# HugoNip/ORB_SLAM2_test

Hardware: AMD Instinct MI355X
Metric: frames/sec ORB extract+match, 1241×376 2000feat 8lvl, 1/2/4/8 GPU (higher is better)
Workload: dtype u8; 1 GPU; C3 KITTI03-shaped mono 1241x376, 2000 feat, 8 lvl: ORBextractor + Hamming knn2 (t vs t-1) + SearchForInitialization(w=100, 0.9, checkOri); global_batch=1024, width=1241, pipelined_batches=True, serial_pass_only=False, input_blocks=4, height=376, nfeatures=2000, nlevels=8

## Files before the change

orb_slam2_test_amd/csrc/blur_device.h:

```cpp
#pragma once

#include <hip/hip_runtime.h>

#include "orbg_internal.h"
#include "orbg_device.h"

#pragma clang fp contract(off)

namespace orbg {

#define BLUR2_TW 244
#define BLUR2_TW_T 240
#ifndef BLUR2_LDS_ROW
#define BLUR2_LDS_ROW 68
#endif
#ifndef ORBG_BLUR2_SEG
#define ORBG_BLUR2_SEG 32
#endif
#ifndef ORBG_BLUR2_ROWPF
#define ORBG_BLUR2_ROWPF 4
#endif

__device__ __forceinline__ uint32_t b2_udot2(uint32_t a, uint32_t b, uint32_t c)
{
    typedef unsigned short u16x2 __attribute__((ext_vector_type(2)));
    return __builtin_amdgcn_udot2(__builtin_bit_cast(u16x2, a), __builtin_bit_cast(u16x2, b), c,
                                  false);
}

__device__ __forceinline__ int b2_reflect101(int i, int n)
{
    i = i < 0 ? -i : i;
    return i >= n ? 2 * n - 2 - i : i;
}

struct Blur2Weights {
    uint32_t K00, K01, K10, K11, K12, K20, K21, K22, K31, K32, E0, E1, E2, k6, c0;
    bool norm256;
    __device__ Blur2Weights(const OrbgGeom *g)
    {
        const uint32_t k0 = g->gk[0], k1 = g->gk[1], k2 = g->gk[2], k3 = g->gk[3],
                       k4 = g->gk[4], k5 = g->gk[5];
        k6 = g->gk[6];
        norm256 = k0 + k1 + k2 + k3 + k4 + k5 + k6 == 256u;
        K00 = k0 << 8 | k1 << 16 | k2 << 24;
        K01 = k3 | k4 << 8 | k5 << 16 | k6 << 24;
        K10 = k0 << 16 | k1 << 24;
        K11 = k2 | k3 << 8 | k4 << 16 | k5 << 24;
        K12 = k6;
        K20 = k0 << 24;
        K21 = k1 | k2 << 8 | k3 << 16 | k4 << 24;
        K22 = k5 | k6 << 8;
        K31 = k0 | k1 << 8 | k2 << 16 | k3 << 24;
        K32 = k4 | k5 << 8 | k6 << 16;
        E0 = k0 | k1 << 16;
        E1 = k2 | k3 << 16;
        E2 = k4 | k5 << 16;
        c0 = norm256 ? (1u << 15) : 0u;
    }
};

template <int SEG, bool NORM256, typename Loader, typename Store>
__device__ __forceinline__ void blur2_column(const Blur2Weights &k, Loader &&load, Store &&store)
{
    constexpr int NR = SEG + 6;
    uint32_t s[NR][4];
    uint32_t P[NR][4];
#pragma unroll
    for (int i = 0; i < NR; i++) {
        uint32_t w0, w1, w2;
        load(i, w0, w1, w2);
        s[i][0] = __builtin_amdgcn_udot4(w1, k.K01, __builtin_amdgcn_udot4(w0, k.K00, 0u, false), false);
        s[i][1] = __builtin_amdgcn_udot4(w2, k.K12, __builtin_amdgcn_udot4(w1, k.K11, __builtin_amdgcn_udot4(w0, k.K10, 0u, false), false), false);
        s[i][2] = __builtin_amdgcn_udot4(w2, k.K22, __builtin_amdgcn_udot4(w1, k.K21, __builtin_amdgcn_udot4(w0, k.K20, 0u, false), false), false);
        s[i][3] = __builtin_amdgcn_udot4(w2, k.K32, __builtin_amdgcn_udot4(w1, k.K31, 0u, false), false);
        if (i >= 1) {
#pragma unroll
            for (int c = 0; c < 4; c++) P[i - 1][c] = s[i - 1][c] | s[i][c] << 16;
        }
        if (i >= 6) {
            const int o = i - 6;
            uint32_t a[4];
#pragma unroll
            for (int c = 0; c < 4; c++) {
                uint32_t v = b2_udot2(P[o][c], k.E0, k.c0);
                v = b2_udot2(P[o + 2][c], k.E1, v);
                v = b2_udot2(P[o + 4][c], k.E2, v);
                a[c] = __umul24(k.k6, s[o + 6][c]) + v;
            }
            uint32_t word;
            if constexpr (NORM256) {
                word = __builtin_amdgcn_perm(a[1], a[0], 0x0c0c0602u) |
                       __builtin_amdgcn_perm(a[3], a[2], 0x06020c0cu);
            } else {
                word = 0;
#pragma unroll
                for (int c = 0; c < 4; c++) word |= min((a[c] + (1u << 15)) >> 16, 255u) << (8 * c);
            }
            store(o, word);
        }
    }
}

template <int SEG, bool TILED = false>
__device__ __forceinline__ void blur2_tile(const Blur2Weights &k, const uint8_t *src, int pitch,
                                           int W, int H, uint8_t *dst, int dpitch, int tx, int y0,
                                           int yend, int lane, uint32_t *wlds = nullptr)
{
    constexpr int PF = ORBG_BLUR2_ROWPF;
    constexpr int TW = TILED ? BLUR2_TW_T : BLUR2_TW;
    static_assert(!TILED || SEG % 8 == 0, "tiled output: whole tile rows per wave");
    const int gx = tx * TW + 4 * lane;
    const bool owner = 4 * lane < TW && gx < W;
    const bool left_wave = tx == 0, right_wave = (tx + 1) * TW + 8 > W;
    const bool is_left = gx == 0;
    const int m = W - gx;
    uint32_t sel1 = 0x07060504u, sel2 = 0x07060504u;
    bool pair_lo = false;
    if (m >= 1 && m <= 7) {
        pair_lo = m <= 3;
        sel1 = sel2 = 0;
#pragma unroll
        for (int b = 4; b < 12; b++) {
            int sb = b < m + 4 ? b : 2 * m + 6 - b;
            if (b >= 8) sb = pair_lo ? max(sb, 0) : max(sb, 4) - 4;
            else sb = max(sb, 0);
            if (b < 8) sel1 |= (uint32_t)sb << (8 * (b - 4));
            else sel2 |= (uint32_t)sb << (8 * (b - 8));
        }
    }
    const int nrec = (H - 1) * pitch + W;
    const int sh0 = (int)((uintptr_t)src & 3);
    const __amdgpu_buffer_rsrc_t rsrc = __builtin_amdgcn_make_buffer_rsrc(
        (void *)(src - sh0), (short)0, nrec + sh0, 0x00020000);
    bool strad_wave;
    {
        const int ro = (H - 1) * pitch;
        const int ol = ro - ((ro + sh0) & 3) + gx - 4;
        strad_wave = __ballot(ol + 4 > nrec && ol < nrec) != 0;
    }
    const __amdgpu_buffer_rsrc_t drsrc = __builtin_amdgcn_make_buffer_rsrc(
        (void *)dst, (short)0, (TILED ? (yend + 7) & ~7 : yend) * dpitch, 0x00020000);
    const int lane_off = owner ? gx : (1 << 30);
    const bool interior = y0 >= 3 && y0 + SEG + 3 < H;
    auto run = [&](auto INTERIOR, auto NORM) {
        constexpr bool inner = decltype(INTERIOR)::value;
        uint32_t ring[PF], rsh[PF];
        auto issue = [&](int i) {
            const int y = inner ? y0 - 3 + i : b2_reflect101(min(y0 - 3 + i, H + 2), H);
            const int rowoff = y * pitch;
            const int sh = __builtin_amdgcn_readfirstlane((rowoff + sh0) & 3);
            const int o = rowoff - sh + gx - 4;
            uint32_t v;
            v = __builtin_amdgcn_raw_buffer_load_b32(rsrc, o + sh0, 0, 0);
            if (!inner && strad_wave && y == H - 1) {
                if (o + 4 > nrec && o < nrec) {
                    uint32_t vb = 0;
                    for (int b = 0; b < 4 && o + b < nrec; b++)
                        vb |= (uint32_t)__builtin_amdgcn_raw_buffer_load_b8(rsrc, o + b + sh0, 0, 0) << (8 * b);
                    v = vb;
                }
            }
            ring[i % PF] = v;
            rsh[i % PF] = (uint32_t)sh;
        };
#pragma unroll
        for (int i = 0; i < PF; i++) issue(i);
        blur2_column<SEG, decltype(NORM)::value>(
            k,
            [&](int i, uint32_t &w0, uint32_t &w1, uint32_t &w2) {
                const uint32_t d0 = ring[i % PF], sh = rsh[i % PF];
                if (i + PF < SEG + 6) issue(i + PF);
                const uint32_t d1 = __builtin_amdgcn_mov_dpp(d0, 0x130, 0xF, 0xF, true);
                const uint32_t d2 = __builtin_amdgcn_mov_dpp(d1, 0x130, 0xF, 0xF, true);
                const uint32_t d3 = __builtin_amdgcn_mov_dpp(d2, 0x130, 0xF, 0xF, true);
                w0 = __builtin_amdgcn_alignbyte(d1, d0, sh);
                w1 = __builtin_amdgcn_alignbyte(d2, d1, sh);
                w2 = __builtin_amdgcn_alignbyte(d3, d2, sh);
                if (left_wave) {
                    const uint32_t r = __builtin_amdgcn_perm(w2, w1, 0x01020304u);
                    w0 = is_left ? r : w0;
                }
                if (right_wave) {
                    const uint32_t v1 = __builtin_amdgcn_perm(w1, w0, sel1);
                    const uint32_t v2 = pair_lo ? __builtin_amdgcn_perm(w1, w0, sel2)
                                                : __builtin_amdgcn_perm(w2, w1, sel2);
                    w1 = v1;
                    w2 = v2;
                }
            },
            [&](int o, uint32_t word) {
                if (!TILED) {
                    __builtin_amdgcn_raw_buffer_store_b32(word, drsrc, lane_off + (y0 + o) * dpitch,
                                                          0, 0);
                    return;
                }
                wlds[(o & 7) * BLUR2_LDS_ROW + lane] = word;
                if ((o & 7) != 7) return;
                wave_sync_lds();
                const int tyoff = ((y0 + (o & ~7)) >> 3) * (8 * dpitch);
#pragma unroll
                for (int h = 0; h < 2; h++) {
                    const int idx = lane + 64 * h, t = idx >> 3, r = idx & 7;
                    typedef uint32_t b2_v4u __attribute__((ext_vector_type(4)));
                    const b2_v4u v = *(const b2_v4u *)(wlds + r * BLUR2_LDS_ROW + 4 * t);
                    const int x = tx * TW + 16 * t;
                    const int off = (t < TW / 16 && x < W) ? tyoff + (x >> 4) * 128 + r * 16 : (1 << 30);
                    __builtin_amdgcn_raw_buffer_store_b128(v, drsrc, off, 0, 0);
                }
                wave_sync_lds();
            });
    };
    if (k.norm256) {
        if (interior)
            run(std::true_type{}, std::true_type{});
        else
            run(std::false_type{}, std::true_type{});
    } else {
        if (interior)
            run(std::true_type{}, std::false_type{});
        else
            run(std::false_type{}, std::false_type{});
    }
}

}
```

orb_slam2_test_amd/csrc/match_kernels.hip:

```cpp
#include <hip/hip_runtime.h>

#include <algorithm>
#include <climits>

#include "../../include/orbg.h"
#include "orbg_internal.h"
#include "orbg_device.h"
#include "match_device.h"

#pragma clang fp contract(off)

namespace orbg {

void prof_begin(void *prof, hipStream_t s, const char *n, hipEvent_t *a);
void prof_end(void *prof, hipStream_t s, const char *n, hipEvent_t a);
bool prof_skip_name(const char *n);

#ifndef ORBG_ROW16_SHFL
__device__ __forceinline__ int row16_sum(int x)
{
    x += __builtin_amdgcn_mov_dpp(x, 0x128, 0xf, 0xf, false);
    x += __builtin_amdgcn_mov_dpp(x, 0x124, 0xf, 0xf, false);
    x += __builtin_amdgcn_mov_dpp(x, 0x4e, 0xf, 0xf, false);
    x += __builtin_amdgcn_mov_dpp(x, 0xb1, 0xf, 0xf, false);
    return x;
}
__device__ __forceinline__ unsigned long long row16_min_u64(unsigned long long v)
{
    auto step = [&](auto CTRL) {
        constexpr int c = decltype(CTRL)::value;
        const uint32_t lo = __builtin_amdgcn_mov_dpp((int)(uint32_t)v, c, 0xf, 0xf, false);
        const uint32_t hi = __builtin_amdgcn_mov_dpp((int)(uint32_t)(v >> 32), c, 0xf, 0xf, false);
        const unsigned long long u = (unsigned long long)hi << 32 | lo;
        v = u < v ? u : v;
    };
    step(std::integral_constant<int, 0x128>{});
    step(std::integral_constant<int, 0x124>{});
    step(std::integral_constant<int, 0x4e>{});
    step(std::integral_constant<int, 0xb1>{});
    return v;
}
#else
__device__ __forceinline__ int row16_sum(int x)
{
#pragma unroll
    for (int o = 8; o > 0; o >>= 1) x += __shfl_xor(x, o, 16);
    return x;
}
__device__ __forceinline__ unsigned long long row16_min_u64(unsigned long long mn)
{
#pragma unroll
    for (int o = 8; o > 0; o >>= 1) {
        const unsigned long long u = __shfl_xor(mn, o, 16);
        mn = u < mn ? u : mn;
    }
    return mn;
}
#endif

#define TH_LOW 50
#define HISTO_LENGTH 30

typedef int knn_v4i __attribute__((ext_vector_type(4)));
typedef int knn_v16i __attribute__((ext_vector_type(16)));

#define KNN_MAX_TRAIN 8192
#define KNN_NONE 0x40000000

__device__ __forceinline__ void knn_key_update(int key, int &k1, int &k2)
{
    k2 = min(k2, max(k1, key));
    k1 = min(k1, key);
}

typedef int knn_v8i __attribute__((ext_vector_type(8)));
typedef float knn_v16f __attribute__((ext_vector_type(16)));
#ifndef ORBG_KNN_MED3
#define ORBG_KNN_MED3 1
#endif
#define KNN4_ROWB 144
#define KNN4_SCALE_A (127 + 12)
#define KNN4_SCALE_B 127

__device__ __forceinline__ uint32_t knn4_neg(uint32_t x, int q)
{
    return (((x >> q) & 0x11111111u) << 3) | 0x22222222u;
}
__device__ __forceinline__ uint32_t knn4_pos(uint32_t x, int q)
{
    return knn4_neg(x, q) ^ 0x88888888u;
}

__device__ __forceinline__ void knn2_block_fp4(const uint8_t *__restrict__ q, int nq,
                                               const uint8_t *__restrict__ t, int nt,
                                               int32_t *__restrict__ out, int qbase)
{
    __shared__ __attribute__((aligned(16))) uint8_t tile[2][64 * KNN4_ROWB];
    const int tid = threadIdx.x, lane = tid & 63, wv = tid >> 6;
    const int col = lane & 31, h = lane >> 5;
    knn_v8i bq[2][4];
#pragma unroll
    for (int u = 0; u < 2; u++) {
        const int qi = qbase + wv * 64 + u * 32 + col;
        uint32_t x[4] = {0, 0, 0, 0};
        if (qi < nq) {
            const uint32_t *p = (const uint32_t *)(q + (size_t)qi * 32);
#pragma unroll
            for (int s = 0; s < 4; s++) x[s] = p[2 * s + h];
        }
#pragma unroll
        for (int s = 0; s < 4; s++) {
#pragma unroll
            for (int qd = 0; qd < 4; qd++) {
                bq[u][s][qd] = (int)knn4_pos(x[s], qd);
                bq[u][s][qd + 4] = 0;
            }
        }
    }
    uint32_t k1[2] = {UINT_MAX, UINT_MAX}, k2[2] = {UINT_MAX, UINT_MAX};

    const int er = tid >> 3, esd = tid & 7;
    auto fetch1 = [&](int row) -> uint32_t {
        return ((const uint32_t *)(t + (size_t)min(row, nt - 1) * 32))[esd];
    };
    auto expand1 = [&](uint32_t x, uint8_t *dst) {
        uint4 w;
        w.x = knn4_neg(x, 0); w.y = knn4_neg(x, 1);
        w.z = knn4_neg(x, 2); w.w = knn4_neg(x, 3);
        *(uint4 *)dst = w;
    };
    auto expand = [&](uint32_t x0, uint32_t x1, int bf) {
        expand1(x0, tile[bf] + er * KNN4_ROWB + esd * 16);
        expand1(x1, tile[bf] + (er + 32) * KNN4_ROWB + esd * 16);
    };
    uint32_t xr0 = 0, xr1 = 0;
    if (nt > 0) {
        expand(fetch1(er), fetch1(er + 32), 0);
        xr0 = fetch1(64 + er);
        xr1 = fetch1(96 + er);
    }
    knn_v16f accA[2], accB[2];
    auto epilogue = [&](const knn_v16f (&acc)[2]) {
#pragma unroll
        for (int r = 0; r < 16; r++) {
#pragma unroll
            for (int u = 0; u < 2; u++) {
                const float kf = acc[u][r];
                const uint32_t key = __float_as_uint(kf);
#if ORBG_KNN_MED3
                const uint32_t k1o = k1[u];
                k1[u] = min(k1o, key);
                asm volatile("v_med3_u32 %0, %1, %2, %3" : "=v"(k2[u]) : "v"(k1o), "v"(k2[u]), "v"(key));
#else
                k2[u] = min(k2[u], max(k1[u], key));
                k1[u] = min(k1[u], key);
#endif
            }
        }
    };
    auto subtile = [&](int tb, int bf, int sub, knn_v16f (&acc)[2]) {
        knn_v16f ctag;
        const float tbh = (float)(tb + 4 * h + (1 << 20));
#pragma unroll
        for (int r = 0; r < 16; r++) ctag[r] = tbh + (float)((r & 3) + 8 * (r >> 2));
        if (tb + 32 > nt) {
#pragma unroll
            for (int r = 0; r < 16; r++)
                if (ctag[r] >= (float)(nt + (1 << 20))) ctag[r] = (float)KNN_NONE;
        }
        const uint8_t *arow = tile[bf] + (32 * sub + col) * KNN4_ROWB + h * 16;
#pragma unroll
        for (int s = 0; s < 4; s++) {
            const knn_v4i a4 = *(const knn_v4i *)(arow + s * 32);
            const knn_v8i a = {a4[0], a4[1], a4[2], a4[3], 0, 0, 0, 0};
            acc[0] = __builtin_amdgcn_mfma_scale_f32_32x32x64_f8f6f4(
                a, bq[0][s], s ? acc[0] : ctag, 4, 4, 0, KNN4_SCALE_A, 0, KNN4_SCALE_B);
            acc[1] = __builtin_amdgcn_mfma_scale_f32_32x32x64_f8f6f4(
                a, bq[1][s], s ? acc[1] : ctag, 4, 4, 0, KNN4_SCALE_A, 0, KNN4_SCALE_B);
        }
    };
    bool pendB = false;
    for (int s0 = 0, bf = 0; s0 < nt; s0 += 64, bf ^= 1) {
        __syncthreads();
        if (s0 + 64 < nt) {
            expand(xr0, xr1, bf ^ 1);
            xr0 = fetch1(s0 + 128 + er);
            xr1 = fetch1(s0 + 160 + er);
        }
        subtile(s0, bf, 0, accA);
        if (pendB) epilogue(accB);
        pendB = s0 + 32 < nt;
        if (pendB) subtile(s0 + 32, bf, 1, accB);
        epilogue(accA);
    }
    if (pendB) epilogue(accB);
    const uint32_t none = 0x4E000000u;
#pragma unroll
    for (int u = 0; u < 2; u++) {
        const uint32_t o1 = (uint32_t)__shfl_xor((int)k1[u], 32, 64);
        const uint32_t o2 = (uint32_t)__shfl_xor((int)k2[u], 32, 64);
        const uint32_t b1 = min(k1[u], o1);
        const uint32_t b2 = min(min(k2[u], o2), max(k1[u], o1));
        const int qi = qbase + wv * 64 + u * 32 + col;
        if (h == 0 && qi < nq) {
            const bool v1 = b1 < none, v2 = b2 < none;
            const int e1 = v1 ? (int)__builtin_bit_cast(float, b1) : 0;
            const int e2 = v2 ? (int)__builtin_bit_cast(float, b2) : 0;
            out[(size_t)qi * 3 + 0] = v1 ? (e1 & (KNN_MAX_TRAIN - 1)) : -1;
            out[(size_t)qi * 3 + 1] = v1 ? (e1 >> 13) : INT_MAX;
            out[(size_t)qi * 3 + 2] = v2 ? (e2 >> 13) : INT_MAX;
        }
    }
}

__global__ __launch_bounds__(256) __attribute__((amdgpu_waves_per_eu(4, 8))) void k_knn2_single(
    const uint8_t *q, int nq, const uint8_t *t, int nt, int32_t *out)
{
    knn2_block_fp4(q, nq, t, nt, out, blockIdx.x * 256);
}

#define KNN2_PAIRS_BODY(BLOCK)                                                                 \
    const int nbx = (fc + 255) >> 8;                                                           \
    const int id = xcd_remap(blockIdx.x, gridDim.x);                                           \
    const int p = id / nbx, bx = id - p * nbx;                                                 \
    const int a = f1[p], b = f2[p];                                                            \
    const int nq = counts[b], nt = counts[a];                                                  \
    if (bx * 256 >= nq) return;                                                                \
    BLOCK(desc + (size_t)b * fc * 32, nq, desc + (size_t)a * fc * 32, nt,                      \
          out + (size_t)p * fc * 3, bx * 256);
__global__ __launch_bounds__(256) __attribute__((amdgpu_waves_per_eu(4, 8))) void k_knn2_pairs(
    const uint8_t *desc, const int32_t *counts, int fc, const int32_t *f1, const int32_t *f2,
    int32_t *out)
{
    KNN2_PAIRS_BODY(knn2_block_fp4)
}

struct F2Key {
    float x, y;
    int idx;
};

#ifndef INIT_QPW
#define INIT_QPW 8
#endif
#ifndef INIT_QPW_SINGLE
#define INIT_QPW_SINGLE 4
#endif
#define INIT_F2_CAP 4608

__host__ __device__ constexpr size_t init_cands_keys_bytes(int f2cap)
{
    return ((size_t)2 * f2cap * sizeof(F2Key) + 15) & ~(size_t)15;
}
#ifndef ORBG_INIT_LDSD
#define ORBG_INIT_LDSD 1
#endif
__host__ __device__ constexpr bool init_cands_lds(int f2cap)
{
    return ORBG_INIT_LDSD && init_cands_keys_bytes(f2cap) + (size_t)f2cap * 32 <= 65536;
}

template <bool LDSD, int QPW>
__device__ __forceinline__ void init_cands_block(const orbg_keypoint *__restrict__ k1,
                                 const uint8_t *__restrict__ d1, int n1,
                                 const orbg_keypoint *__restrict__ k2,
                                 const uint8_t *__restrict__ d2, int n2, orbg_bounds b,
                                 const float *__restrict__ prev, int prev_stride, int window,
                                 unsigned long long *__restrict__ topk, int32_t *__restrict__ topn,
                                 int qbase, int f2cap)
{
    extern __shared__ __attribute__((aligned(16))) F2Key f2mem[];
    F2Key *f2raw = f2mem, *f2 = f2mem + f2cap;
    uint4 *d2l = (uint4 *)((uint8_t *)f2mem + init_cands_keys_bytes(f2cap));
    __shared__ int nf2;
    __shared__ int colstart[ORBG_GRID_COLS + 1];
    const int tid = threadIdx.x, lane = tid & 63, wv = tid >> 6;
    const GridPrm g = grid_prm(b);
    if (tid == 0) nf2 = 0;
    if (tid <= ORBG_GRID_COLS) colstart[tid] = 0;
    __syncthreads();
    const int n2s = min(n2, f2cap);
    if (LDSD) {
        const uint4 *src = (const uint4 *)d2;
        for (int i0 = 0; i0 < 2 * n2s; i0 += 4 * 256) {
            uint4 v[4];
#pragma unroll
            for (int u = 0; u < 4; u++) {
                const int i = i0 + u * 256 + tid;
                v[u] = src[i < 2 * n2s ? i : 0];
            }
#pragma unroll
            for (int u = 0; u < 4; u++) {
                const int i = i0 + u * 256 + tid;
                if (i < 2 * n2s) d2l[i] = v[u];
            }
        }
    }
    for (int i = tid; i < n2s; i += 256) {
        const orbg_keypoint kp = k2[i];
        if (kp.octave == 0) {
            const int px = (int)roundf((kp.x - g.min_x) * g.inv_w);
            if (px < 0 || px >= ORBG_GRID_COLS) continue;
            const int s = atomicAdd(&nf2, 1);
            if (s < f2cap) {
                f2raw[s] = F2Key{kp.x, kp.y, i};
                atomicAdd(&colstart[px + 1], 1);
            }
        }
    }
    __syncthreads();
    const int m = min(nf2, f2cap);
    if (wv == 0) {
        const int c = colstart[lane + 1];
        const int incl = wave_incl_scan(c);
        colstart[lane + 1] = incl;
    }
    __syncthreads();
    __shared__ int cursor[ORBG_GRID_COLS];
    if (tid < ORBG_GRID_COLS) cursor[tid] = colstart[tid];
    __syncthreads();
    for (int j = tid; j < m; j += 256) {
        const F2Key fk = f2raw[j];
        const int px = (int)roundf((fk.x - g.min_x) * g.inv_w);
        f2[atomicAdd(&cursor[px], 1)] = fk;
    }
    __syncthreads();
    const float r = (float)window;
    const int grp = lane >> 4, sub = lane & 15;
    for (int qq = 0; qq < QPW; qq += 4) {
        const int i1 = qbase + wv * QPW + qq + grp;
        bool act = i1 < n1;
        if (act && k1[i1].octave > 0) {
            if (sub == 0) topn[i1] = -1;
            act = false;
        }
        if (!__any(act)) continue;
        unsigned long long loc[ORBG_MATCH_TOPK];
#pragma unroll
        for (int k = 0; k < ORBG_MATCH_TOPK; k++) loc[k] = ~0ull;
        int cnt = 0;
        if (act) {
            const Window w = make_window(g, prev[(size_t)i1 * prev_stride],
                                         prev[(size_t)i1 * prev_stride + 1], r);
            uint32_t qd[8];
            {
                const uint4 *p = (const uint4 *)(d1 + (size_t)i1 * 32);
                const uint4 a = p[0], c = p[1];
                qd[0] = a.x; qd[1] = a.y; qd[2] = a.z; qd[3] = a.w;
                qd[4] = c.x; qd[5] = c.y; qd[6] = c.z; qd[7] = c.w;
            }
            if (!w.empty) {
                const int j0 = colstart[w.cx0], j1 = colstart[w.cx1 + 1];
                for (int j = j0 + sub; j < j1; j += 16) {
                    const F2Key fk = f2[j];
                    const int ord = cand_order(g, w, fk.x, fk.y);
                    if (ord < 0) continue;
                    const int d = LDSD ? hamming8(qd, (const uint32_t *)(d2l + 2 * fk.idx))
                                       : hamming8(qd, (const uint32_t *)(d2 + (size_t)fk.idx * 32));
                    unsigned long long key = ((unsigned long long)d << 32) |
                                             ((unsigned long long)ord << 20) | (unsigned)fk.idx;
                    cnt++;
#pragma unroll
                    for (int k = 0; k < ORBG_MATCH_TOPK; k++) {
                        const unsigned long long lo = key < loc[k] ? key : loc[k];
                        const unsigned long long hi = key < loc[k] ? loc[k] : key;
                        loc[k] = lo;
                        key = hi;
                    }
                }
            }
        }
        cnt = row16_sum(cnt);
        int head = 0;
        unsigned long long *out = topk + (size_t)i1 * ORBG_MATCH_TOPK;
        for (int k = 0; k < ORBG_MATCH_TOPK; k++) {
            unsigned long long mine = ~0ull;
#pragma unroll
            for (int h = 0; h < ORBG_MATCH_TOPK; h++)
                if (h == head) mine = loc[h];
            const unsigned long long mn = row16_min_u64(mine);
            if (mn != ~0ull && mine == mn) head++;
            if (act && sub == 0) out[k] = mn;
        }
        if (act && sub == 0) topn[i1] = cnt;
    }
}

template <bool LDSD>
__global__ __launch_bounds__(256) void k_init_cands_single(
    const orbg_keypoint *k1, const uint8_t *d1, int n1, const orbg_keypoint *k2,
    const uint8_t *d2, int n2, orbg_bounds b, const float *prev, int window,
    unsigned long long *topk, int32_t *topn)
{
    init_cands_block<LDSD, INIT_QPW_SINGLE>(k1, d1, n1, k2, d2, n2, b, prev, 2, window, topk, topn,
                                            blockIdx.x * 4 * INIT_QPW_SINGLE, n2);
}

template <bool LDSD>
__global__ __launch_bounds__(256) void k_init_cands_pairs(
    const orbg_keypoint *kps, const uint8_t *desc, const int32_t *counts, int fc,
    const int32_t *f1, const int32_t *f2, orbg_bounds b, int window, unsigned long long *topk,
    int32_t *topn, int cap)
{
    const int nbx = (cap + 4 * INIT_QPW - 1) / (4 * INIT_QPW);
    const int id = xcd_remap(blockIdx.x, gridDim.x);
    const int p = id / nbx, bx = id - p * nbx;
    const int a = f1[p], c = f2[p];
    const int n1 = counts[a], n2 = counts[c];
    const int qbase = bx * 4 * INIT_QPW;
    if (qbase >= n1) return;
    const orbg_keypoint *k1 = kps + (size_t)a * fc;
    if (k1[qbase].octave > 0) {
        for (int i = qbase + threadIdx.x; i < min(n1, qbase + 4 * INIT_QPW); i += 256)
            topn[(size_t)p * fc + i] = -1;
        return;
    }
    init_cands_block<LDSD, INIT_QPW>(k1, desc + (size_t)a * fc * 32, n1, kps + (size_t)c * fc,
                     desc + (size_t)c * fc * 32, n2, b, (const float *)k1,
                     (int)(sizeof(orbg_keypoint) / sizeof(float)), window,
                     topk + (size_t)p * fc * ORBG_MATCH_TOPK, topn + (size_t)p * fc, qbase, cap);
}

#define RESOLVE_CHUNK 64
#define RESOLVE_N2_CAP 4608

struct ResolveShared {
    unsigned long long (*chunk)[RESOLVE_CHUNK * ORBG_MATCH_TOPK];
    int (*chunkn)[RESOLVE_CHUNK];
    int nbuf;
    int *hsize;
    int *nmp;
    float *ang1, *ang2;
    uint16_t *mdist;
    int16_t *m21, *m12;
    int8_t *hbin;
    int32_t *owner;
};

#define RESOLVE_CHUNK_BYTES (RESOLVE_CHUNK * ORBG_MATCH_TOPK * 8 + RESOLVE_CHUNK * 4)
#define RESOLVE_FIXED_BYTES (32 * 4 + 16)

#ifndef RESOLVE_PRELOAD
#define RESOLVE_PRELOAD 0
#endif
#define RESOLVE_PRELOAD_CAP 1024

__host__ __device__ constexpr int resolve_nbuf(int cap, bool single)
{
    return (RESOLVE_PRELOAD >= (single ? 1 : 2) && cap <= RESOLVE_PRELOAD_CAP)
               ? (cap + RESOLVE_CHUNK - 1) / RESOLVE_CHUNK > 2 ? (cap + RESOLVE_CHUNK - 1) / RESOLVE_CHUNK : 2
               : 2;
}

__host__ __device__ constexpr size_t resolve_lds_bytes(int cap, int nbuf)
{
    return (size_t)nbuf * RESOLVE_CHUNK_BYTES + RESOLVE_FIXED_BYTES + (size_t)cap * 8 +
           (((size_t)cap * 7 + 15) & ~(size_t)15) + (size_t)cap * 4;
}

__device__ __forceinline__ ResolveShared resolve_layout(uint8_t *base, int cap, int nbuf)
{
    ResolveShared S;
    S.nbuf = nbuf;
    S.chunk = (unsigned long long(*)[RESOLVE_CHUNK * ORBG_MATCH_TOPK])base;
    base += (size_t)nbuf * RESOLVE_CHUNK * ORBG_MATCH_TOPK * 8;
    S.chunkn = (int(*)[RESOLVE_CHUNK])base;
    base += (size_t)nbuf * RESOLVE_CHUNK * 4;
    S.hsize = (int *)base;
    base += 32 * 4;
    S.nmp = (int *)base;
    base += 16;
    S.ang1 = (float *)base;
    S.ang2 = S.ang1 + cap;
    base += (size_t)cap * 8;
    S.mdist = (uint16_t *)base;
    S.m21 = (int16_t *)(S.mdist + cap);
    S.m12 = S.m21 + cap;
    S.hbin = (int8_t *)(S.m12 + cap);
    S.owner = (int32_t *)(base + (((size_t)cap * 7 + 15) & ~(size_t)15));
    return S;
}

#ifdef ORBG_DEV_KNOBS
__device__ unsigned long long g_rprof[8];
#define RP_NOW() __builtin_readcyclecounter()
#define RP_ADD(k, v)                                                                         \
    do {                                                                                     \
        if (threadIdx.x == 0) atomicAdd(&g_rprof[k], (unsigned long long)(v));               \
    } while (0)
#else
#define RP_NOW() 0ull
#define RP_ADD(k, v) \
    do {             \
    } while (0)
#endif

__device__ void rescan(const orbg_keypoint *k2, const uint8_t *d2, int n2, const GridPrm &g,
                       const Window &w, const uint32_t qd[8], const uint16_t *mdist, int *best,
                       int *best2, int *bidx)
{
// ... 315 lines not shown
    RP_ADD(4, RP_NOW() - rp_t);
}

__global__ __launch_bounds__(RESOLVE_T) void k_init_resolve_single(
    const orbg_keypoint *k1, const uint8_t *d1, int n1, const orbg_keypoint *k2,
    const uint8_t *d2, int n2, orbg_bounds b, const float *prev, float *prev_out, int window,
    float nnratio, int check_ori, const unsigned long long *topk, const int32_t *topn,
    int32_t *m12, int32_t *nm, int cap)
{
    extern __shared__ __attribute__((aligned(16))) uint8_t rs_lds[];
    ResolveShared S = resolve_layout(rs_lds, cap, resolve_nbuf(cap, true));
    init_resolve_block(S, cap, k1, d1, n1, k2, d2, n2, b, prev, 2, window, nnratio, check_ori, topk,
                       topn, m12, nm, prev_out);
}

__global__ __launch_bounds__(RESOLVE_T) void k_init_resolve_pairs(
    const orbg_keypoint *kps, const uint8_t *desc, const int32_t *counts, int fc,
    const int32_t *f1, const int32_t *f2, orbg_bounds b, int window, float nnratio,
    int check_ori, const unsigned long long *topk, const int32_t *topn, int32_t *m12,
    int32_t *nm, int cap)
{
    extern __shared__ __attribute__((aligned(16))) uint8_t rs_lds[];
    ResolveShared S = resolve_layout(rs_lds, cap, resolve_nbuf(cap, false));
    const int p = blockIdx.x;
    const int a = f1[p], c = f2[p];
    const orbg_keypoint *k1 = kps + (size_t)a * fc;
    init_resolve_block(S, cap, k1, desc + (size_t)a * fc * 32, counts[a], kps + (size_t)c * fc,
                      desc + (size_t)c * fc * 32, counts[c], b, (const float *)k1,
                      (int)(sizeof(orbg_keypoint) / sizeof(float)), window, nnratio, check_ori,
                      topk + (size_t)p * fc * ORBG_MATCH_TOPK, topn + (size_t)p * fc,
                      m12 + (size_t)p * fc, nm + p, nullptr);
}

#define PL(prof, st, name, ...)                                                            \
    do {                                                                                   \
        if (prof_skip_name(name)) break;                                                   \
        hipEvent_t a_ = nullptr;                                                           \
        prof_begin(prof, st, name, &a_);                                                   \
        __VA_ARGS__;                                                                       \
        prof_end(prof, st, name, a_);                                                      \
    } while (0)

__global__ __launch_bounds__(256) void k_match_export(const int32_t *__restrict__ m12,
                                                      const int32_t *__restrict__ f1,
                                                      const int32_t *__restrict__ counts,
                                                      int frame_cap, int npairs,
                                                      int32_t *__restrict__ out)
{
    const int64_t i = (int64_t)blockIdx.x * 256 + threadIdx.x;
    if (i >= (int64_t)npairs * frame_cap) return;
    const int p = (int)(i / frame_cap), k = (int)(i - (int64_t)p * frame_cap);
    out[i] = k < counts[f1[p]] ? m12[i] : -1;
}

int launch_match_export(hipStream_t st, const int32_t *m12, const int32_t *f1,
                        const int32_t *counts, int frame_cap, int npairs, int32_t *out)
{
    const int64_t n = (int64_t)npairs * frame_cap;
    if (n <= 0) return ORBG_OK;
    hipLaunchKernelGGL(k_match_export, dim3((unsigned)((n + 255) / 256)), dim3(256), 0, st, m12,
                       f1, counts, frame_cap, npairs, out);
    return hipGetLastError() == hipSuccess ? ORBG_OK : ORBG_EIO;
}

int launch_knn2(hipStream_t st, const uint8_t *q, int nq, const uint8_t *t, int nt, int32_t *out,
                void *prof)
{
    if (nt >= KNN_MAX_TRAIN) return ORBG_ENOTSUP;
    PL(prof, st, "knn2",
       hipLaunchKernelGGL(k_knn2_single,
                          dim3((nq + 255) / 256), dim3(256), 0, st, q, nq, t, nt, out));
    return hipGetLastError() == hipSuccess ? ORBG_OK : ORBG_EIO;
}

int launch_match_pairs(hipStream_t st, hipStream_t aux, hipEvent_t evf, hipEvent_t evj,
                       const uint8_t *desc, const orbg_keypoint *kps,
                       const int32_t *counts, int fc, const int32_t *d_f1, const int32_t *d_f2,
                       int npairs, orbg_bounds b, int window, float nnratio, int check_ori,
                       int32_t *knn, int32_t *m12, int32_t *nm, uint32_t *topk, int32_t *topk_n,
                       void *prof, int serial, int cap0)
{
    if (fc > RESOLVE_N2_CAP || fc > (1 << 20) || cap0 > fc) return ORBG_ENOTSUP;
    PL(prof, st, "init_cands",
       hipLaunchKernelGGL(k_init_cands_pairs<false>,
                          dim3((cap0 + 4 * INIT_QPW - 1) / (4 * INIT_QPW) * npairs), dim3(256),
                          init_cands_keys_bytes(cap0), st, kps, desc, counts, fc, d_f1, d_f2, b,
                          window, (unsigned long long *)topk, topk_n, cap0));
    if (serial) aux = st;
    if (hipEventRecord(evf, st) != hipSuccess || hipStreamWaitEvent(aux, evf, 0) != hipSuccess)
        return ORBG_EIO;
    PL(prof, aux, "knn2",
       hipLaunchKernelGGL(k_knn2_pairs,
                          dim3((fc + 255) / 256 * npairs), dim3(256), 0, aux, desc, counts, fc,
                          d_f1, d_f2, knn));
    if (hipEventRecord(evj, aux) != hipSuccess) return ORBG_EIO;
    if (resolve_lds_bytes(cap0, resolve_nbuf(cap0, false)) > 65536) {
        static bool pattr = false;
        if (!pattr) {
            if (hipFuncSetAttribute((const void *)k_init_resolve_pairs,
                                    hipFuncAttributeMaxDynamicSharedMemorySize,
                                    (int)resolve_lds_bytes(RESOLVE_PRELOAD_CAP,
                                                           resolve_nbuf(RESOLVE_PRELOAD_CAP, false))) !=
                hipSuccess)
                return ORBG_EIO;
            pattr = true;
        }
    }
    PL(prof, st, "init_resolve",
       hipLaunchKernelGGL(k_init_resolve_pairs, dim3(npairs), dim3(RESOLVE_T),
                          resolve_lds_bytes(cap0, resolve_nbuf(cap0, false)), st, kps, desc,
                          counts, fc, d_f1, d_f2, b,
                          window, nnratio, check_ori, (const unsigned long long *)topk, topk_n,
                          m12, nm, cap0));
    if (hipStreamWaitEvent(st, evj, 0) != hipSuccess) return ORBG_EIO;
    return hipGetLastError() == hipSuccess ? ORBG_OK : ORBG_EIO;
}

#ifdef ORBG_DEV_KNOBS
extern "C" int orbg_dev_resolve_prof(unsigned long long out[8], int reset)
{
    if (hipMemcpyFromSymbol(out, HIP_SYMBOL(g_rprof), sizeof(g_rprof)) != hipSuccess) return -5;
    if (reset) {
        const unsigned long long z[8] = {0, 0, 0, 0, 0, 0, 0, 0};
        if (hipMemcpyToSymbol(HIP_SYMBOL(g_rprof), z, sizeof(z)) != hipSuccess) return -5;
    }
    return 0;
}
#endif

int launch_init_match_single(hipStream_t st, const orbg_keypoint *k1, const uint8_t *d1, int n1,
                             const orbg_keypoint *k2, const uint8_t *d2, int n2, orbg_bounds b,
                             const float *prev, float *prev_out, int32_t *m12, int32_t *nm,
                             int window, float nnratio,
                             int check_ori, uint32_t *topk, int32_t *topk_n, void *prof, int cap)
{
    const int nq = std::min(n1, cap), n2c = std::min(n2, cap);
    if (n1 > RESOLVE_N2_CAP || n2 > RESOLVE_N2_CAP || n2 > INIT_F2_CAP) return ORBG_ENOTSUP;
    static bool attr = false;
    if (!attr) {
        if (hipFuncSetAttribute((const void *)k_init_resolve_single,
                                hipFuncAttributeMaxDynamicSharedMemorySize,
                                (int)std::max(resolve_lds_bytes(RESOLVE_N2_CAP, 2),
                                              resolve_lds_bytes(RESOLVE_PRELOAD_CAP,
                                                                resolve_nbuf(RESOLVE_PRELOAD_CAP, true)))) !=
                hipSuccess)
            return ORBG_EIO;
        attr = true;
    }
    PL(prof, st, "init_cands",
       if (init_cands_lds(std::max(n2c, 1)))
           hipLaunchKernelGGL(k_init_cands_single<true>,
                              dim3((nq + 4 * INIT_QPW_SINGLE - 1) / (4 * INIT_QPW_SINGLE)), dim3(256),
                              init_cands_keys_bytes(std::max(n2c, 1)) + (size_t)std::max(n2c, 1) * 32,
                              st, k1, d1, nq, k2, d2, n2c, b, prev, window,
                              (unsigned long long *)topk, topk_n);
       else
           hipLaunchKernelGGL(k_init_cands_single<false>,
                              dim3((nq + 4 * INIT_QPW_SINGLE - 1) / (4 * INIT_QPW_SINGLE)), dim3(256),
                              init_cands_keys_bytes(std::max(n2c, 1)), st, k1, d1, nq, k2, d2, n2c,
                              b, prev, window, (unsigned long long *)topk, topk_n));
    PL(prof, st, "init_resolve",
       hipLaunchKernelGGL(k_init_resolve_single, dim3(1), dim3(RESOLVE_T),
                          resolve_lds_bytes(cap, resolve_nbuf(cap, true)), st, k1, d1, n1, k2, d2,
                          n2, b, prev, prev_out, window,
                          nnratio, check_ori, (const unsigned long long *)topk, topk_n, m12, nm,
                          cap));
    return hipGetLastError() == hipSuccess ? ORBG_OK : ORBG_EIO;
}

}
// ... 1 lines not shown
```

orb_slam2_test_amd/csrc/pyramid_kernels.hip:

```cpp
#include <hip/hip_runtime.h>

#include "orbg_device.h"
#include "blur_device.h"
#include "pyramid_args.h"

#pragma clang fp contract(off)

namespace orbg {

__device__ __forceinline__ uint32_t pyr_dot2(uint32_t a, uint32_t b)
{
    typedef unsigned short u16x2 __attribute__((ext_vector_type(2)));
    return __builtin_amdgcn_udot2(__builtin_bit_cast(u16x2, a), __builtin_bit_cast(u16x2, b), 0u,
                                  false);
}

__device__ __forceinline__ uint32_t pyr_mulhi(uint32_t h16, uint32_t b8)
{
    const uint32_t x = h16 & 0x00FFFF00u, y = b8 & 0x000FFFFFu;
    return (uint32_t)(((unsigned long long)x * y) >> 32);
}

struct PyrOct {
    uint32_t sel[PYR_COLS], cf[PYR_COLS];
};

__device__ __forceinline__ void pyr_hrow(uint4 raw, uint32_t o, const PyrOct &t,
                                         uint32_t h[PYR_COLS])
{
    const uint32_t w0 = __builtin_amdgcn_alignbyte(raw.y, raw.x, o);
    const uint32_t w1 = __builtin_amdgcn_alignbyte(raw.z, raw.y, o);
    const uint32_t w2 = __builtin_amdgcn_alignbyte(raw.w, raw.z, o);
#pragma unroll
    for (int i = 0; i < 4; i++) h[i] = pyr_dot2(__builtin_amdgcn_perm(w1, w0, t.sel[i]), t.cf[i]);
#pragma unroll
    for (int i = 4; i < 8; i++) h[i] = pyr_dot2(__builtin_amdgcn_perm(w2, w1, t.sel[i]), t.cf[i]);
}

__device__ __forceinline__ uint4 pyr_load(const uint8_t *p, const uint8_t *end, bool guard,
                                          uint32_t &o)
{
    o = (uint32_t)(uintptr_t)p & 3u;
    const uint8_t *a = p - o;
    if (guard && a + 16 > end) {
        uint32_t w[4] = {0, 0, 0, 0};
        for (int b = 0; b < 16; b++)
            if (a + b < end) w[b >> 2] |= (uint32_t)a[b] << (8 * (b & 3));
        return make_uint4(w[0], w[1], w[2], w[3]);
    }
    return *(const uint4 *)a;
}

__device__ __forceinline__ void pyr_oct(const uint4 *__restrict__ oct, PyrOct &t)
{
    const uint4 s0 = oct[1], s1 = oct[2], c0 = oct[3], c1 = oct[4];
    t.sel[0] = s0.x; t.sel[1] = s0.y; t.sel[2] = s0.z; t.sel[3] = s0.w;
    t.sel[4] = s1.x; t.sel[5] = s1.y; t.sel[6] = s1.z; t.sel[7] = s1.w;
    t.cf[0] = c0.x; t.cf[1] = c0.y; t.cf[2] = c0.z; t.cf[3] = c0.w;
    t.cf[4] = c1.x; t.cf[5] = c1.y; t.cf[6] = c1.z; t.cf[7] = c1.w;
}

__device__ __forceinline__ void pyr_wave_item(const uint8_t *__restrict__ src, int spitch,
                                              uint8_t *__restrict__ dst, int dpitch,
                                              const int4 *__restrict__ ytab,
                                              const uint4 *__restrict__ oct, int dx0, bool store,
                                              int y0, int n)
{
    PyrOct t;
    pyr_oct(oct, t);
    const int sx0 = (int)oct[0].x;
    int4 yt = ytab[y0];
    const int first = yt.x & 0xFFFF;
    const int nsrc = (ytab[y0 + n - 1].x >> 16) - first + 1;
    const uint8_t *rp = src + (int64_t)first * spitch + sx0;
    uint4 ring[PYR_PF];
    uint32_t oring[PYR_PF];
#pragma unroll
    for (int p = 0; p < PYR_PF; p++)
        ring[p] = pyr_load(rp + (int64_t)min(p, nsrc - 1) * spitch, nullptr, false, oring[p]);
    uint32_t h[2][PYR_COLS];
#pragma unroll
    for (int i = 0; i < PYR_COLS; i++) h[1][i] = 0;
    int k = 0, nexty = (yt.x >> 16) - first;
    uint8_t *drow = dst + (int64_t)y0 * dpitch + dx0;
#pragma unroll
    for (int j = 0; j < PYR_NS; j++) {
        uint32_t *hc = h[j & 1], *hp = h[(j & 1) ^ 1];
        const uint4 raw = ring[j % PYR_PF];
        const uint32_t o = oring[j % PYR_PF];
        if (j + PYR_PF < PYR_NS)
            ring[j % PYR_PF] = pyr_load(rp + (int64_t)min(j + PYR_PF, nsrc - 1) * spitch,
                                        nullptr, false, oring[j % PYR_PF]);
        pyr_hrow(raw, o, t, hc);
#pragma unroll
        for (int i = 0; i < PYR_COLS; i++) hc[i] &= 0x00FFFF00u;
        if (j == nexty) {
            const uint32_t y8 = (uint32_t)yt.y & 0x000FFFFFu, z8 = (uint32_t)yt.z & 0x000FFFFFu;
            uint32_t v[PYR_COLS];
#pragma unroll
            for (int i = 0; i < PYR_COLS; i++) {
                const uint32_t a = (uint32_t)(((unsigned long long)hp[i] * y8) >> 32);
                const uint32_t b = (uint32_t)(((unsigned long long)hc[i] * z8) >> 32);
                v[i] = (a + b + 2) >> 2;
            }
            const uint32_t lo = v[0] | v[1] << 8 | v[2] << 16 | v[3] << 24;
            const uint32_t hi = v[4] | v[5] << 8 | v[6] << 16 | v[7] << 24;
            if ((yt.x & 0xFFFF) - first != j && store)
                *(uint2 *)drow = make_uint2(lo, hi);
            drow += dpitch;
            k++;
            yt = ytab[y0 + min(k, n - 1)];
            nexty = k < n ? (yt.x >> 16) - first : 1 << 30;
        }
    }
}

__device__ __forceinline__ void pyr_fix(const uint8_t *src, int spitch, uint8_t *dst,
                                        int dpitch, int dw, const int4 *ytab, const uint4 *oct,
                                        int dx0, int dy, const uint8_t *end, bool guard)
{
    PyrOct t;
    pyr_oct(oct, t);
    const uint4 o0 = oct[0];
    const int4 yt = ytab[dy];
    uint32_t h0[PYR_COLS], h1[PYR_COLS];
    {
        uint32_t o;
        uint4 raw = pyr_load(src + (int64_t)(yt.x & 0xFFFF) * spitch + (int)o0.x, end, guard, o);
        pyr_hrow(raw, o, t, h0);
        raw = pyr_load(src + (int64_t)(yt.x >> 16) * spitch + (int)o0.x, end, guard, o);
        pyr_hrow(raw, o, t, h1);
    }
    const uint32_t b0 = (uint32_t)yt.w & 0xFFFFu, b1 = (uint32_t)yt.w >> 16;
    uint8_t *d = dst + (int64_t)dy * dpitch + dx0;
    const int nc = min(PYR_COLS, dw - dx0);
#pragma unroll
    for (int i = 0; i < PYR_COLS; i++) {
        uint32_t v;
        if (o0.y >> i & 1u) {
            v = ((h0[i] >> 4) * b0 + (h1[i] >> 4) * b1 + (1u << 21)) >> 22;
        } else {
            const uint32_t a = (uint32_t)(((unsigned long long)(h0[i] & 0x00FFFF00u) *
                                           ((uint32_t)yt.y & 0x000FFFFFu)) >> 32);
            const uint32_t b = (uint32_t)(((unsigned long long)(h1[i] & 0x00FFFF00u) *
                                           ((uint32_t)yt.z & 0x000FFFFFu)) >> 32);
            v = (a + b + 2) >> 2;
        }
        if (i < nc) d[i] = (uint8_t)v;
    }
}

__global__ __launch_bounds__(1024) void k_pyramid(PyrArgs A, const OrbgGeom *__restrict__ g,
                                                 const uint4 *__restrict__ ptab,
                                                 const int4 *__restrict__ ytab_all,
                                                 const int4 *__restrict__ bands,
                                                 const uint8_t *__restrict__ img0,
                                                 int64_t img_fs, int img_pitch,
                                                 const uint8_t *img_end, uint8_t *pyr,
                                                 uint8_t *blur, int nframes)
{
    const int id = xcd_remap(blockIdx.x, gridDim.x);
    const int f = id / A.nband, band = id - f * A.nband;
    const int lane = threadIdx.x & 63;
    const int wv = __builtin_amdgcn_readfirstlane(threadIdx.x >> 6);
    const int nw = blockDim.x >> 6;
    uint8_t *fpyr = pyr + (int64_t)f * A.pyr_frame;
    for (int ph = 0; ph < A.L; ph++) {
        const int l = ph + 1;
        if (l < A.L) {
            const PyrLevelArgs &P = A.lv[l];
            const bool lvl1 = l == 1;
            const uint8_t *src = lvl1 ? img0 + (int64_t)f * img_fs : fpyr + P.src_off;
            const int spitch = lvl1 ? img_pitch : P.spitch;
            uint8_t *dst = fpyr + P.dst_off;
            const int4 cr = bands[band * A.L + l];
            const int4 *ytab = ytab_all + P.ytab_off;
// ... 61 lines not shown
```

Before: 194,700 frames/s.

## Pack init-candidate keys into 32 bits, add triple med3 KNN epilogue, direct-load blur/pyramid paths

Adds a 32-bit packed top-k key path for the initialization candidate kernel. It is selected when the candidate cap fits in 11 bits and replaces 64-bit compares and DPP reductions with 32-bit ones, widening the key back to 64 bits on output. The KNN epilogue now processes accumulator rows in triples, using v_med3 to update the best-two keys with fewer operations. Blur and pyramid kernels gain unaligned 12-byte direct-load paths, but both are behind macros that default to 0, so only the key32 and triple epilogue paths run by default.

```diff
diff --git a/orb_slam2_test_amd/csrc/blur_device.h b/orb_slam2_test_amd/csrc/blur_device.h
--- a/orb_slam2_test_amd/csrc/blur_device.h
+++ b/orb_slam2_test_amd/csrc/blur_device.h
@@ -16,6 +16,9 @@
 #endif
 #ifndef ORBG_BLUR2_SEG
 #define ORBG_BLUR2_SEG 32
+#endif
+#ifndef ORBG_BLUR2_DIRECT
+#define ORBG_BLUR2_DIRECT 0
 #endif
 #ifndef ORBG_BLUR2_ROWPF
 #define ORBG_BLUR2_ROWPF 4
@@ -143,6 +146,27 @@
         (void *)dst, (short)0, (TILED ? (yend + 7) & ~7 : yend) * dpitch, 0x00020000);
     const int lane_off = owner ? gx : (1 << 30);
     const bool interior = y0 >= 3 && y0 + SEG + 3 < H;
+    auto store_row = [&](int o, uint32_t word) {
+        if (!TILED) {
+            __builtin_amdgcn_raw_buffer_store_b32(word, drsrc, lane_off + (y0 + o) * dpitch,
+                                                  0, 0);
+            return;
+        }
+        wlds[(o & 7) * BLUR2_LDS_ROW + lane] = word;
+        if ((o & 7) != 7) return;
+        wave_sync_lds();
+        const int tyoff = ((y0 + (o & ~7)) >> 3) * (8 * dpitch);
+#pragma unroll
+        for (int h = 0; h < 2; h++) {
+            const int idx = lane + 64 * h, t = idx >> 3, r = idx & 7;
+            typedef uint32_t b2_v4u __attribute__((ext_vector_type(4)));
+            const b2_v4u v = *(const b2_v4u *)(wlds + r * BLUR2_LDS_ROW + 4 * t);
+            const int x = tx * TW + 16 * t;
+            const int off = (t < TW / 16 && x < W) ? tyoff + (x >> 4) * 128 + r * 16 : (1 << 30);
+            __builtin_amdgcn_raw_buffer_store_b128(v, drsrc, off, 0, 0);
+        }
+        wave_sync_lds();
+    };
     auto run = [&](auto INTERIOR, auto NORM) {
         constexpr bool inner = decltype(INTERIOR)::value;
         uint32_t ring[PF], rsh[PF];
@@ -189,28 +213,40 @@
                     w2 = v2;
                 }
             },
-            [&](int o, uint32_t word) {
-                if (!TILED) {
-                    __builtin_amdgcn_raw_buffer_store_b32(word, drsrc, lane_off + (y0 + o) * dpitch,
-                                                          0, 0);
-                    return;
-                }
-                wlds[(o & 7) * BLUR2_LDS_ROW + lane] = word;
-                if ((o & 7) != 7) return;
-                wave_sync_lds();
-                const int tyoff = ((y0 + (o & ~7)) >> 3) * (8 * dpitch);
-#pragma unroll
-                for (int h = 0; h < 2; h++) {
-                    const int idx = lane + 64 * h, t = idx >> 3, r = idx & 7;
-                    typedef uint32_t b2_v4u __attribute__((ext_vector_type(4)));
-                    const b2_v4u v = *(const b2_v4u *)(wlds + r * BLUR2_LDS_ROW + 4 * t);
-                    const int x = tx * TW + 16 * t;
-                    const int off = (t < TW / 16 && x < W) ? tyoff + (x >> 4) * 128 + r * 16 : (1 << 30);
-                    __builtin_amdgcn_raw_buffer_store_b128(v, drsrc, off, 0, 0);
-                }
-                wave_sync_lds();
-            });
+            store_row);
     };
+#if ORBG_BLUR2_DIRECT
+    auto run_direct = [&](auto NORM) {
+        typedef uint32_t b2_v3u __attribute__((ext_vector_type(3)));
+        typedef b2_v3u b2_v3u_ua __attribute__((aligned(1)));
+        b2_v3u ring[PF];
+        const uint32_t xoff = (uint32_t)(gx - 4);
+        auto issue = [&](int i) {
+            const uint8_t *row = src + (int64_t)(y0 - 3 + i) * pitch;
+            ring[i % PF] = *(const b2_v3u_ua *)(row + xoff);
+        };
+#pragma unroll
+        for (int i = 0; i < PF; i++) issue(i);
+        blur2_column<SEG, decltype(NORM)::value>(
+            k,
+            [&](int i, uint32_t &w0, uint32_t &w1, uint32_t &w2) {
+                const b2_v3u v = ring[i % PF];
+                if (i + PF < SEG + 6) issue(i + PF);
+                __builtin_amdgcn_sched_barrier(0);
+                w0 = v.x;
+                w1 = v.y;
+                w2 = v.z;
+            },
+            store_row);
+    };
+    if (interior && !left_wave && !right_wave) {
+        if (k.norm256)
+            run_direct(std::true_type{});
+        else
+            run_direct(std::false_type{});
+        return;
+    }
+#endif
     if (k.norm256) {
         if (interior)
             run(std::true_type{}, std::true_type{});
diff --git a/orb_slam2_test_amd/csrc/match_kernels.hip b/orb_slam2_test_amd/csrc/match_kernels.hip
--- a/orb_slam2_test_amd/csrc/match_kernels.hip
+++ b/orb_slam2_test_amd/csrc/match_kernels.hip
@@ -2,6 +2,7 @@
 
 #include <algorithm>
 #include <climits>
+#include <type_traits>
 
 #include "../../include/orbg.h"
 #include "orbg_internal.h"
@@ -40,7 +41,21 @@
     step(std::integral_constant<int, 0xb1>{});
     return v;
 }
+__device__ __forceinline__ uint32_t row16_min_u32(uint32_t v)
+{
+    v = min(v, (uint32_t)__builtin_amdgcn_mov_dpp((int)v, 0x128, 0xf, 0xf, false));
+    v = min(v, (uint32_t)__builtin_amdgcn_mov_dpp((int)v, 0x124, 0xf, 0xf, false));
+    v = min(v, (uint32_t)__builtin_amdgcn_mov_dpp((int)v, 0x4e, 0xf, 0xf, false));
+    v = min(v, (uint32_t)__builtin_amdgcn_mov_dpp((int)v, 0xb1, 0xf, 0xf, false));
+    return v;
+}
 #else
+__device__ __forceinline__ uint32_t row16_min_u32(uint32_t mn)
+{
+#pragma unroll
+    for (int o = 8; o > 0; o >>= 1) mn = min(mn, (uint32_t)__shfl_xor((int)mn, o, 16));
+    return mn;
+}
 __device__ __forceinline__ int row16_sum(int x)
 {
 #pragma unroll
@@ -77,6 +92,9 @@
 typedef float knn_v16f __attribute__((ext_vector_type(16)));
 #ifndef ORBG_KNN_MED3
 #define ORBG_KNN_MED3 1
+#endif
+#ifndef ORBG_KNN_TRIPLE
+#define ORBG_KNN_TRIPLE 1
 #endif
 #define KNN4_ROWB 144
 #define KNN4_SCALE_A (127 + 12)
@@ -141,8 +159,28 @@
     }
     knn_v16f accA[2], accB[2];
     auto epilogue = [&](const knn_v16f (&acc)[2]) {
+#if ORBG_KNN_TRIPLE && ORBG_KNN_MED3
+#pragma unroll
+        for (int r = 0; r + 2 < 16; r += 3) {
+#pragma unroll
+            for (int u = 0; u < 2; u++) {
+                const float fa = acc[u][r], fb = acc[u][r + 1], fc = acc[u][r + 2];
+                const uint32_t a = __float_as_uint(fa), b = __float_as_uint(fb),
+                               c = __float_as_uint(fc);
+                const uint32_t lo = min(min(a, b), c);
+                uint32_t md;
+                asm volatile("v_med3_u32 %0, %1, %2, %3" : "=v"(md) : "v"(a), "v"(b), "v"(c), "v"(lo));
+                const uint32_t t = max(k1[u], lo);
+                k1[u] = min(k1[u], lo);
+                k2[u] = min(min(t, k2[u]), md);
+            }
+        }
+#pragma unroll
+        for (int r = 15; r < 16; r++) {
+#else
 #pragma unroll
         for (int r = 0; r < 16; r++) {
+#endif
 #pragma unroll
             for (int u = 0; u < 2; u++) {
                 const float kf = acc[u][r];
@@ -260,7 +298,31 @@
     return ORBG_INIT_LDSD && init_cands_keys_bytes(f2cap) + (size_t)f2cap * 32 <= 65536;
 }
 
-template <bool LDSD, int QPW>
+#ifndef ORBG_INIT_KEY32
+#define ORBG_INIT_KEY32 1
+#endif
+#define INIT_K32_IDX_BITS 11
+#define INIT_K32_ORD_BITS 12
+static_assert(ORBG_GRID_COLS * ORBG_GRID_ROWS <= (1 << INIT_K32_ORD_BITS),
+              "grid order px * ROWS + py in 12 bits");
+static_assert(INIT_K32_IDX_BITS + INIT_K32_ORD_BITS + 9 == 32, "d <= 256 in the top 9 bits");
+static_assert((256ull << (INIT_K32_IDX_BITS + INIT_K32_ORD_BITS) |
+               ((1ull << (INIT_K32_IDX_BITS + INIT_K32_ORD_BITS)) - 1)) < 0xFFFFFFFFull,
+              "every real key below the empty key");
+__host__ __device__ constexpr bool init_cands_key32(int f2cap)
+{
+    return ORBG_INIT_KEY32 && f2cap <= (1 << INIT_K32_IDX_BITS);
+}
+__device__ __forceinline__ unsigned long long init_key_widen(uint32_t k)
+{
+    if (k == ~0u) return ~0ull;
+    const uint32_t d = k >> (INIT_K32_IDX_BITS + INIT_K32_ORD_BITS);
+    const uint32_t ord = (k >> INIT_K32_IDX_BITS) & ((1u << INIT_K32_ORD_BITS) - 1);
+    const uint32_t idx = k & ((1u << INIT_K32_IDX_BITS) - 1);
+    return ((unsigned long long)d << 32) | ((unsigned long long)ord << 20) | idx;
+}
+
+template <bool LDSD, int QPW, bool K32 = false>
 __device__ __forceinline__ void init_cands_block(const orbg_keypoint *__restrict__ k1,
                                  const uint8_t *__restrict__ d1, int n1,
                                  const orbg_keypoint *__restrict__ k2,
@@ -335,9 +397,11 @@
             act = false;
         }
         if (!__any(act)) continue;
-        unsigned long long loc[ORBG_MATCH_TOPK];
-#pragma unroll
-        for (int k = 0; k < ORBG_MATCH_TOPK; k++) loc[k] = ~0ull;
+        typedef typename std::conditional<K32, uint32_t, unsigned long long>::type key_t;
+        const key_t none = (key_t)~(key_t)0;
+        key_t loc[ORBG_MATCH_TOPK];
+#pragma unroll
+        for (int k = 0; k < ORBG_MATCH_TOPK; k++) loc[k] = none;
         int cnt = 0;
         if (act) {
             const Window w = make_window(g, prev[(size_t)i1 * prev_stride],
@@ -357,13 +421,18 @@
                     if (ord < 0) continue;
                     const int d = LDSD ? hamming8(qd, (const uint32_t *)(d2l + 2 * fk.idx))
                                        : hamming8(qd, (const uint32_t *)(d2 + (size_t)fk.idx * 32));
-                    unsigned long long key = ((unsigned long long)d << 32) |
-                                             ((unsigned long long)ord << 20) | (unsigned)fk.idx;
+                    key_t key;
+                    if constexpr (K32)
+                        key = (uint32_t)d << (INIT_K32_IDX_BITS + INIT_K32_ORD_BITS) |
+                              (uint32_t)ord << INIT_K32_IDX_BITS | (uint32_t)fk.idx;
+                    else
+                        key = ((unsigned long long)d << 32) | ((unsigned long long)ord << 20) |
+                              (unsigned)fk.idx;
                     cnt++;
 #pragma unroll
                     for (int k = 0; k < ORBG_MATCH_TOPK; k++) {
-                        const unsigned long long lo = key < loc[k] ? key : loc[k];
-                        const unsigned long long hi = key < loc[k] ? loc[k] : key;
+                        const key_t lo = key < loc[k] ? key : loc[k];
+                        const key_t hi = key < loc[k] ? loc[k] : key;
                         loc[k] = lo;
                         key = hi;
                     }
@@ -374,13 +443,21 @@
         int head = 0;
         unsigned long long *out = topk + (size_t)i1 * ORBG_MATCH_TOPK;
         for (int k = 0; k < ORBG_MATCH_TOPK; k++) {
-            unsigned long long mine = ~0ull;
+            key_t mine = none;
 #pragma unroll
             for (int h = 0; h < ORBG_MATCH_TOPK; h++)
                 if (h == head) mine = loc[h];
-            const unsigned long long mn = row16_min_u64(mine);
-            if (mn != ~0ull && mine == mn) head++;
-            if (act && sub == 0) out[k] = mn;
+            key_t mn;
+            if constexpr (K32)
+                mn = row16_min_u32(mine);
+            else
+                mn = row16_min_u64(mine);
+            if (mn != none && mine == mn) head++;
+            if constexpr (K32) {
+                if (act && sub == 0) out[k] = init_key_widen(mn);
+            } else {
+                if (act && sub == 0) out[k] = mn;
+            }
         }
         if (act && sub == 0) topn[i1] = cnt;
     }
@@ -396,7 +473,7 @@
                                             blockIdx.x * 4 * INIT_QPW_SINGLE, n2);
 }
 
-template <bool LDSD>
+template <bool LDSD, bool K32>
 __global__ __launch_bounds__(256) void k_init_cands_pairs(
     const orbg_keypoint *kps, const uint8_t *desc, const int32_t *counts, int fc,
     const int32_t *f1, const int32_t *f2, orbg_bounds b, int window, unsigned long long *topk,
@@ -415,7 +492,7 @@
             topn[(size_t)p * fc + i] = -1;
         return;
     }
-    init_cands_block<LDSD, INIT_QPW>(k1, desc + (size_t)a * fc * 32, n1, kps + (size_t)c * fc,
+    init_cands_block<LDSD, INIT_QPW, K32>(k1, desc + (size_t)a * fc * 32, n1, kps + (size_t)c * fc,
                      desc + (size_t)c * fc * 32, n2, b, (const float *)k1,
                      (int)(sizeof(orbg_keypoint) / sizeof(float)), window,
                      topk + (size_t)p * fc * ORBG_MATCH_TOPK, topn + (size_t)p * fc, qbase, cap);
@@ -897,10 +974,16 @@
 {
     if (fc > RESOLVE_N2_CAP || fc > (1 << 20) || cap0 > fc) return ORBG_ENOTSUP;
     PL(prof, st, "init_cands",
-       hipLaunchKernelGGL(k_init_cands_pairs<false>,
-                          dim3((cap0 + 4 * INIT_QPW - 1) / (4 * INIT_QPW) * npairs), dim3(256),
-                          init_cands_keys_bytes(cap0), st, kps, desc, counts, fc, d_f1, d_f2, b,
-                          window, (unsigned long long *)topk, topk_n, cap0));
+       if (init_cands_key32(cap0))
+           hipLaunchKernelGGL((k_init_cands_pairs<false, true>),
+                              dim3((cap0 + 4 * INIT_QPW - 1) / (4 * INIT_QPW) * npairs), dim3(256),
+                              init_cands_keys_bytes(cap0), st, kps, desc, counts, fc, d_f1, d_f2, b,
+                              window, (unsigned long long *)topk, topk_n, cap0);
+       else
+           hipLaunchKernelGGL((k_init_cands_pairs<false, false>),
+                              dim3((cap0 + 4 * INIT_QPW - 1) / (4 * INIT_QPW) * npairs), dim3(256),
+                              init_cands_keys_bytes(cap0), st, kps, desc, counts, fc, d_f1, d_f2, b,
+                              window, (unsigned long long *)topk, topk_n, cap0));
     if (serial) aux = st;
     if (hipEventRecord(evf, st) != hipSuccess || hipStreamWaitEvent(aux, evf, 0) != hipSuccess)
         return ORBG_EIO;
diff --git a/orb_slam2_test_amd/csrc/pyramid_kernels.hip b/orb_slam2_test_amd/csrc/pyramid_kernels.hip
--- a/orb_slam2_test_amd/csrc/pyramid_kernels.hip
+++ b/orb_slam2_test_amd/csrc/pyramid_kernels.hip
@@ -25,16 +25,20 @@
     uint32_t sel[PYR_COLS], cf[PYR_COLS];
 };
 
+__device__ __forceinline__ void pyr_hrow3(uint32_t w0, uint32_t w1, uint32_t w2, const PyrOct &t,
+                                          uint32_t h[PYR_COLS])
+{
+#pragma unroll
+    for (int i = 0; i < 4; i++) h[i] = pyr_dot2(__builtin_amdgcn_perm(w1, w0, t.sel[i]), t.cf[i]);
+#pragma unroll
+    for (int i = 4; i < 8; i++) h[i] = pyr_dot2(__builtin_amdgcn_perm(w2, w1, t.sel[i]), t.cf[i]);
+}
+
 __device__ __forceinline__ void pyr_hrow(uint4 raw, uint32_t o, const PyrOct &t,
                                          uint32_t h[PYR_COLS])
 {
-    const uint32_t w0 = __builtin_amdgcn_alignbyte(raw.y, raw.x, o);
-    const uint32_t w1 = __builtin_amdgcn_alignbyte(raw.z, raw.y, o);
-    const uint32_t w2 = __builtin_amdgcn_alignbyte(raw.w, raw.z, o);
-#pragma unroll
-    for (int i = 0; i < 4; i++) h[i] = pyr_dot2(__builtin_amdgcn_perm(w1, w0, t.sel[i]), t.cf[i]);
-#pragma unroll
-    for (int i = 4; i < 8; i++) h[i] = pyr_dot2(__builtin_amdgcn_perm(w2, w1, t.sel[i]), t.cf[i]);
+    pyr_hrow3(__builtin_amdgcn_alignbyte(raw.y, raw.x, o), __builtin_amdgcn_alignbyte(raw.z, raw.y, o),
+              __builtin_amdgcn_alignbyte(raw.w, raw.z, o), t, h);
 }
 
 __device__ __forceinline__ uint4 pyr_load(const uint8_t *p, const uint8_t *end, bool guard,
@@ -51,6 +55,41 @@
     return *(const uint4 *)a;
 }
 
+#ifndef ORBG_PYR_DIRECT
+#define ORBG_PYR_DIRECT 0
+#endif
+struct PyrRow {
+#if ORBG_PYR_DIRECT
+    uint32_t w0, w1, w2;
+#else
+    uint4 raw;
+    uint32_t o;
+#endif
+};
+__device__ __forceinline__ PyrRow pyr_load_fast(const uint8_t *p)
+{
+    PyrRow r;
+#if ORBG_PYR_DIRECT
+    typedef uint32_t pyr_v3u __attribute__((ext_vector_type(3)));
+    typedef pyr_v3u pyr_v3u_ua __attribute__((aligned(1)));
+    const pyr_v3u v = *(const pyr_v3u_ua *)p;
+    r.w0 = v.x;
+    r.w1 = v.y;
+    r.w2 = v.z;
+#else
+    r.raw = pyr_load(p, nullptr, false, r.o);
+#endif
+    return r;
+}
+__device__ __forceinline__ void pyr_hrow_fast(const PyrRow &r, const PyrOct &t, uint32_t h[PYR_COLS])
+{
+#if ORBG_PYR_DIRECT
+    pyr_hrow3(r.w0, r.w1, r.w2, t, h);
+#else
+    pyr_hrow(r.raw, r.o, t, h);
+#endif
+}
+
 __device__ __forceinline__ void pyr_oct(const uint4 *__restrict__ oct, PyrOct &t)
 {
     const uint4 s0 = oct[1], s1 = oct[2], c0 = oct[3], c1 = oct[4];
@@ -73,11 +112,9 @@
     const int first = yt.x & 0xFFFF;
     const int nsrc = (ytab[y0 + n - 1].x >> 16) - first + 1;
     const uint8_t *rp = src + (int64_t)first * spitch + sx0;
-    uint4 ring[PYR_PF];
-    uint32_t oring[PYR_PF];
-#pragma unroll
-    for (int p = 0; p < PYR_PF; p++)
-        ring[p] = pyr_load(rp + (int64_t)min(p, nsrc - 1) * spitch, nullptr, false, oring[p]);
+    PyrRow ring[PYR_PF];
+#pragma unroll
+    for (int p = 0; p < PYR_PF; p++) ring[p] = pyr_load_fast(rp + (int64_t)min(p, nsrc - 1) * spitch);
     uint32_t h[2][PYR_COLS];
 #pragma unroll
     for (int i = 0; i < PYR_COLS; i++) h[1][i] = 0;
@@ -86,12 +123,10 @@
 #pragma unroll
     for (int j = 0; j < PYR_NS; j++) {
         uint32_t *hc = h[j & 1], *hp = h[(j & 1) ^ 1];
-        const uint4 raw = ring[j % PYR_PF];
-        const uint32_t o = oring[j % PYR_PF];
+        const PyrRow raw = ring[j % PYR_PF];
         if (j + PYR_PF < PYR_NS)
-            ring[j % PYR_PF] = pyr_load(rp + (int64_t)min(j + PYR_PF, nsrc - 1) * spitch,
-                                        nullptr, false, oring[j % PYR_PF]);
-        pyr_hrow(raw, o, t, hc);
+            ring[j % PYR_PF] = pyr_load_fast(rp + (int64_t)min(j + PYR_PF, nsrc - 1) * spitch);
+        pyr_hrow_fast(raw, t, hc);
 #pragma unroll
         for (int i = 0; i < PYR_COLS; i++) hc[i] &= 0x00FFFF00u;
         if (j == nexty) {
```

Measured after the change: 196,000 frames/s (median of 6 runs). No clear change (+0.6%).
